# jkulhanek/viewformer

Hardware: AMD Instinct MI355X
Metric: novel views/sec (encode->AR transformer->decode), 128px 6-ctx (higher is better)
Workload: dtype bf16

## Files before the change

### viewformer_amd/csrc/epilogue.h

```cpp
#pragma once
#include "vf_common.h"

template <int EPI, bool HAS_RES, typename OffOut, typename OffRes>
__device__ __forceinline__ void vf_store_tile(const f32x16& acc, float bias, float* __restrict__ out,
                                              const float* __restrict__ res, OffOut off_out, OffRes off_res) {
    float v[16];
    if (HAS_RES) {
        float rr[16];
#pragma unroll
        for (int r = 0; r < 16; ++r) rr[r] = res[off_res(r)];
#pragma unroll
        for (int r = 0; r < 16; ++r) {
            float t = acc[r] + bias;
            if (EPI == 1) t = vf_gelu_erf(t);
            if (EPI == 2) t = vf_gelu_erf_fast(t);
            v[r] = t + rr[r];
        }
    } else {
#pragma unroll
        for (int r = 0; r < 16; ++r) {
            float t = acc[r] + bias;
            if (EPI == 1) t = vf_gelu_erf(t);
            if (EPI == 2) t = vf_gelu_erf_fast(t);
            v[r] = t;
        }
    }
#pragma unroll
    for (int r = 0; r < 16; ++r) out[off_out(r)] = v[r];
}

template <int EPI, bool HAS_RES>
__device__ __forceinline__ void vf_store_tile_ragged(const f32x16& acc, float bias, float* __restrict__ out,
                                                     const float* __restrict__ res, long long ldc, long long ldr,
                                                     int rows_left ) {
    if (rows_left <= 0) return;
    float v[16];
#pragma unroll
    for (int r = 0; r < 16; ++r) {
        const int row = (r & 3) + 8 * (r >> 2);
        float t = acc[r] + bias;
        if (EPI == 1) t = vf_gelu_erf(t);
        if (EPI == 2) t = vf_gelu_erf_fast(t);
        if (HAS_RES) t += res[(long long)(row < rows_left ? row : 0) * ldr];
        v[r] = t;
    }
#pragma unroll
    for (int r = 0; r < 16; ++r) {
        const int row = (r & 3) + 8 * (r >> 2);
        if (row < rows_left) out[(long long)row * ldc] = v[r];
    }
}

template <bool HAS_RES, typename OffOut, typename OffRes, typename Sel, typename S>
__device__ __forceinline__ void vf_store_tile_stats(const f32x16& acc, float bias, float* __restrict__ out,
                                                    const float* __restrict__ res, OffOut off_out, OffRes off_res, Sel sel,
                                                    S (&s)[2], S (&q)[2]) {
    float v[16];
    if (HAS_RES) {
        float rr[16];
#pragma unroll
        for (int r = 0; r < 16; ++r) rr[r] = res[off_res(r)];
#pragma unroll
        for (int r = 0; r < 16; ++r) v[r] = acc[r] + bias + rr[r];
    } else {
#pragma unroll
        for (int r = 0; r < 16; ++r) v[r] = acc[r] + bias;
    }
#pragma unroll
    for (int r = 0; r < 16; ++r) {
        const int k = sel(r);
        s[k] += (S)v[r];
        q[k] += (S)v[r] * (S)v[r];
    }
#pragma unroll
    for (int r = 0; r < 16; ++r) out[off_out(r)] = v[r];
}

template <typename OffOut>
__device__ __forceinline__ void vf_store_tile_pre(const f32x16& acc, float bias, float* __restrict__ out, const float (&rr)[16], OffOut off_out) {
    float v[16];
#pragma unroll
    for (int r = 0; r < 16; ++r) v[r] = acc[r] + bias + rr[r];
#pragma unroll
    for (int r = 0; r < 16; ++r) out[off_out(r)] = v[r];
}
template <typename OffOut, typename Sel, typename S>
__device__ __forceinline__ void vf_store_tile_stats_pre(const f32x16& acc, float bias, float* __restrict__ out, const float (&rr)[16], OffOut off_out,
                                                        Sel sel, S (&s)[2], S (&q)[2]) {
    float v[16];
#pragma unroll
    for (int r = 0; r < 16; ++r) v[r] = acc[r] + bias + rr[r];
#pragma unroll
    for (int r = 0; r < 16; ++r) {
        const int k = sel(r);
        s[k] += (S)v[r];
        q[k] += (S)v[r] * (S)v[r];
    }
#pragma unroll
    for (int r = 0; r < 16; ++r) out[off_out(r)] = v[r];
}

template <typename S>
__device__ __forceinline__ void vf_gn_group_reduce(S& s, S& q, int cg) {
    s += __shfl_xor(s, 32, 64);
    q += __shfl_xor(q, 32, 64);
    for (int o = 1; o < cg; o <<= 1) {
        s += __shfl_xor(s, o, 64);
        q += __shfl_xor(q, o, 64);
    }
}
```

### viewformer_amd/csrc/gemm_bf16_g256.hip

```cpp
#include "vf_common.h"
#include "epilogue.h"
#include "../../include/vf_hip.h"

namespace {

typedef __bf16 bf16x8 __attribute__((ext_vector_type(8)));
typedef __bf16 bf16x2_t __attribute__((ext_vector_type(2)));

constexpr int GM = 256, GN = 256, GK = 64;
constexpr int GA_BYTES = GM * GK * 2;
constexpr int GB_BYTES = GN * GK * 2;
constexpr int GSTAGE = GA_BYTES + GB_BYTES;

__device__ __forceinline__ void bufds16(__amdgpu_buffer_rsrc_t r, void* l, unsigned voff, unsigned soff) {
    __builtin_amdgcn_raw_ptr_buffer_load_lds(r, (__attribute__((address_space(3))) void*)l, 16, voff, soff, 0, 0);
}

template <bool DROP, int IC>
__device__ __forceinline__ void g256_store_f32(const vf_igemm_args& p, const f32x16 (&acc)[IC][2], int m_tile0, int n_tile0, int wrow0,
                                               int wave_n, int half, int l31, bool full, bool gelu) {
    const long long ldc = p.ldc, ldr = p.ldr;
    const bool has_res = p.res != nullptr;
    const bool dual = p.epilogue == VF_EPI_GELU_DUAL;
    const int odd = l31 & 1;
    const uint32_t drop_thresh = vf_dropout_thresh(p.drop_rate), drop_key = vf_dropout_key(p.drop_seed, p.drop_site, 0u);
    const float drop_scale = 1.0f / (1.0f - p.drop_rate);
#pragma unroll
    for (int j = 0; j < 2; ++j) {
        const int n = n_tile0 + wave_n * 64 + j * 32 + l31;
        const float bias = p.bias ? p.bias[n] : 0.f;
#pragma unroll
        for (int i = 0; i < IC; ++i) {
            int m0 = m_tile0 + wrow0 + i * 32 + 4 * half;
            if constexpr (DROP) asm volatile("" : "+v"(m0) :: "memory");
            const int rows_left = p.M - m0;
            float* o = p.out + (size_t)(rows_left > 0 ? m0 : 0) * ldc + n;
            float v[16];
#pragma unroll
            for (int r = 0; r < 16; ++r) v[r] = acc[i][j][r] + bias;
            if (gelu) {
#pragma unroll
                for (int r = 0; r < 16; ++r) v[r] = vf_gelu_erf_fast(v[r]);
            }
            if constexpr (DROP) {
#pragma unroll
                for (int g = 0; g < 4; ++g) {
                    const uint32_t w = vf_dropout_word(drop_key, (uint32_t)(((m0 + p.drop_row0) >> 2) + 2 * g) * (uint32_t)p.Cout + (uint32_t)n);
#pragma unroll
                    for (int e = 0; e < 4; ++e) v[4 * g + e] = vf_dropout_keep(w, e, drop_thresh) ? v[4 * g + e] * drop_scale : 0.f;
                }
            }
            if (has_res) {
                const float* rs = p.res + (size_t)(rows_left > 0 ? m0 : 0) * ldr + n;
                float rr[16];
#pragma unroll
                for (int r = 0; r < 16; ++r) {
                    const int row = (r & 3) + 8 * (r >> 2);
                    rr[r] = rs[(long long)(full || row < rows_left ? row : 0) * ldr];
                }
#pragma unroll
                for (int r = 0; r < 16; ++r) v[r] += rr[r];
            }
            if (full) {
#pragma unroll
                for (int r = 0; r < 16; ++r) o[(long long)((r & 3) + 8 * (r >> 2)) * ldc] = v[r];
            } else if (rows_left > 0) {
#pragma unroll
                for (int r = 0; r < 16; ++r) {
                    const int row = (r & 3) + 8 * (r >> 2);
                    if (row < rows_left) o[(long long)row * ldc] = v[r];
                }
            }
            if (dual) {
                __builtin_amdgcn_sched_barrier(0);
                __bf16* o16 = reinterpret_cast<__bf16*>(p.out_aux) + (size_t)(rows_left > 0 ? m0 : 0) * ldc + (n - odd);
#pragma unroll
                for (int r = 0; r < 16; ++r) v[r] = vf_gelu_erf_fast(v[r]);
#pragma unroll
                for (int r = 0; r < 16; r += 2) {
                    const float give = odd ? v[r] : v[r + 1];
                    const float got = vf_lane_xor1(give);
                    const int row = ((r + odd) & 3) + 8 * ((r + odd) >> 2);
                    bf16x2_t h;
                    h[0] = (__bf16)(odd ? got : v[r]);
                    h[1] = (__bf16)(odd ? v[r + 1] : got);
                    if (full || row < rows_left) *reinterpret_cast<bf16x2_t*>(o16 + (long long)row * ldc) = h;
                }
            }
            __builtin_amdgcn_sched_barrier(0);
        }
    }
}

template <int EPI, bool FULL, int IC>
__device__ __forceinline__ void g256_store_bf16(const vf_igemm_args& p, const f32x16 (&acc)[IC][2], int m_tile0, int n_tile0, int wrow0,
                                                int wave_n, int half, int l31) {
    __bf16* __restrict__ O = reinterpret_cast<__bf16*>(p.out);
    const int odd = l31 & 1;
#pragma unroll
    for (int j = 0; j < 2; ++j) {
        const int n = n_tile0 + wave_n * 64 + j * 32 + l31;
        const float bias = p.bias ? p.bias[n] : 0.f;
#pragma unroll
        for (int i = 0; i < IC; ++i) {
            const int m0 = m_tile0 + wrow0 + i * 32 + 4 * half;
            float t[16];
            if (EPI == 2 || EPI == 4) {
                const bool u16 = p.reserved0 & 4;
                const unsigned esz = u16 ? 2u : 4u;
                const __amdgpu_buffer_rsrc_t u_rs = __builtin_amdgcn_make_buffer_rsrc(
                    const_cast<unsigned char*>(reinterpret_cast<const unsigned char*>(p.res) + (size_t)m_tile0 * p.ldr * esz), 0,
                    (int)min((long long)0x7fffffff, (long long)(p.M - m_tile0) * p.ldr * esz), 0x00020000);
                float uu[16];
                if (u16) {
                    const unsigned voff = ((unsigned)(m0 - m_tile0) * (unsigned)p.ldr + (unsigned)(n - odd)) * 2u;
                    unsigned w[8];
#pragma unroll
                    for (int r = 0; r < 16; r += 2) {
                        const int row = ((r + odd) & 3) + 8 * ((r + odd) >> 2);
                        w[r >> 1] = __builtin_amdgcn_raw_buffer_load_b32(u_rs, voff + (unsigned)row * (unsigned)p.ldr * 2u, 0, 0);
                    }
#pragma unroll
                    for (int r = 0; r < 16; r += 2) {
                        const unsigned mine = w[r >> 1];
                        const unsigned give = odd ? (mine << 16) : (mine & 0xffff0000u);
                        const unsigned got = vf_lane_xor1(give);
                        uu[r] = __builtin_bit_cast(float, odd ? got : (mine << 16));
                        uu[r + 1] = __builtin_bit_cast(float, odd ? (mine & 0xffff0000u) : got);
                    }
                } else {
                    const unsigned voff = ((unsigned)(m0 - m_tile0) * (unsigned)p.ldr + (unsigned)n) * 4u;
#pragma unroll
                    for (int r = 0; r < 16; ++r) {
                        const unsigned soff = (unsigned)((r & 3) + 8 * (r >> 2)) * (unsigned)p.ldr * 4u;
                        uu[r] = __builtin_bit_cast(float, __builtin_amdgcn_raw_buffer_load_b32(u_rs, voff, soff, 0));
                    }
                }
                __builtin_amdgcn_sched_barrier(0);
#pragma unroll
                for (int q = 0; q < 4; ++q) {
#pragma unroll
                    for (int e = 0; e < 4; ++e)
                        t[4 * q + e] = __fmul_rn(__fadd_rn(acc[i][j][4 * q + e], bias), EPI == 4 ? uu[4 * q + e] : vf_gelu_grad_fast(uu[4 * q + e]));
                    __builtin_amdgcn_sched_barrier(0);
                }
            } else {
#pragma unroll
                for (int r = 0; r < 16; ++r) {
                    t[r] = acc[i][j][r] + bias;
                    if (EPI == 1) t[r] = vf_gelu_erf_fast(t[r]);
                }
            }
            float gq[EPI == 5 ? 16 : 1];
            if (EPI == 5) {
#pragma unroll
                for (int r = 0; r < 16; ++r) { float f, g; vf_gelu_and_grad_fast(t[r], f, g); t[r] = f; gq[r] = g; }
            }
#pragma unroll
            for (int pass = 0; pass < ((EPI == 3 || EPI == 5) ? 2 : 1); ++pass) {
                __bf16* __restrict__ dst = pass == 0 ? O : reinterpret_cast<__bf16*>(p.out_aux);
                if (EPI == 3 && pass == 1) {
                    __builtin_amdgcn_sched_barrier(0);
#pragma unroll
                    for (int r = 0; r < 16; ++r) t[r] = vf_gelu_erf_fast(t[r]);
                }
#pragma unroll
                for (int r = 0; r < 16; r += 2) {
                    const float lo = (EPI == 5 && pass == 0) ? gq[r] : t[r], hi = (EPI == 5 && pass == 0) ? gq[r + 1] : t[r + 1];
                    const float give = odd ? lo : hi;
                    const float got = vf_lane_xor1(give);
                    const int m = m0 + ((r + odd) & 3) + 8 * ((r + odd) >> 2);
                    bf16x2_t v;
                    v[0] = (__bf16)(odd ? got : lo);
                    v[1] = (__bf16)(odd ? hi : got);
                    if (FULL || m < p.M) *reinterpret_cast<bf16x2_t*>(dst + (size_t)m * p.ldc + (n - odd)) = v;
                }
            }
        }
    }
}

template <bool O16, bool DROP, int IC>
__device__ __forceinline__ void g256_tile(const vf_igemm_args& p, unsigned char* smem_b, int m_tile0, int nblk, int tid) {
    constexpr int TROWS = 2 * IC * 32;
    const int lane = tid & 63;
    const int wave = __builtin_amdgcn_readfirstlane(tid >> 6);
    const int wave_m = wave >> 2, wave_n = wave & 3;
    const int half = lane >> 5, l31 = lane & 31;
    const int wrow0 = wave_m * (IC * 32);
    const int n_tile0 = nblk * GN;
    const int nstages = p.Cin / GK;

    const bool a_mover = wave * 32 < TROWS;
    const __amdgpu_buffer_rsrc_t a_rsrc = __builtin_amdgcn_make_buffer_rsrc(const_cast<float*>(p.x), 0, 0x7fffffff, 0x00020000);
    const __amdgpu_buffer_rsrc_t w_rsrc = __builtin_amdgcn_make_buffer_rsrc(const_cast<float*>(p.w_packed), 0, 0x7fffffff, 0x00020000);
    unsigned avoff[4];
#pragma unroll
    for (int q = 0; q < 4; ++q) {
        const int r = wave * 32 + q * 8 + (lane >> 3);
        const int c = (lane & 7) ^ ((r >> 1) & 7);
        int m = m_tile0 + r;
        m = m < p.M ? m : p.M - 1;
        avoff[q] = (unsigned)(((size_t)m * p.lda) * 2 + c * 16);
    }
    const unsigned wvoff = (unsigned)((size_t)nblk * GB_BYTES + wave * 4096 + lane * 16);
    const size_t w_stage_stride = (size_t)(p.Cout / 128) * (GK * 128 * 2);
    auto issue = [&](int s) {
        unsigned char* dst = smem_b + (s & 1) * GSTAGE;
        if (IC == 4 || a_mover) {
#pragma unroll
            for (int q = 0; q < 4; ++q) bufds16(a_rsrc, dst + (wave * 32 + q * 8) * 128, avoff[q], (unsigned)(s * (GK * 2)));
        }
#pragma unroll
        for (int q = 0; q < 4; ++q) bufds16(w_rsrc, dst + GA_BYTES + wave * 4096 + q * 1024, wvoff + q * 1024, (unsigned)((size_t)s * w_stage_stride));
    };

    const unsigned a_row_off = (unsigned)((wrow0 + l31) * 128);
    const unsigned a_swz = (unsigned)((l31 >> 1) & 7);
    unsigned a_off[4];
#pragma unroll
    for (int ks = 0; ks < 4; ++ks) a_off[ks] = a_row_off + ((((unsigned)(ks * 2 + half)) ^ a_swz) << 4);
    const unsigned b_off = (unsigned)(GA_BYTES + (wave_n >> 1) * (GK * 128 * 2) + ((half * 128) + (wave_n & 1) * 64 + l31) * 16);

    f32x16 acc[IC][2];
#pragma unroll
    for (int i = 0; i < IC; ++i)
#pragma unroll
        for (int j = 0; j < 2; ++j)
#pragma unroll
            for (int r = 0; r < 16; ++r) acc[i][j][r] = 0.f;

    issue(0);
    for (int s = 0; s < nstages; ++s) {
        asm volatile("s_waitcnt vmcnt(0) lgkmcnt(0)" ::: "memory");
        __builtin_amdgcn_s_barrier();
        if (s + 1 < nstages) issue(s + 1);
        const unsigned char* buf = smem_b + (s & 1) * GSTAGE;
        bf16x8 a[2][IC], b[2][2];
        auto frags = [&](int ks, bf16x8 (&af)[IC], bf16x8 (&bf)[2]) {
#pragma unroll
            for (int j = 0; j < 2; ++j) bf[j] = *reinterpret_cast<const bf16x8*>(buf + b_off + (ks * 2 * 128 + j * 32) * 16);
#pragma unroll
            for (int i = 0; i < IC; ++i) af[i] = *reinterpret_cast<const bf16x8*>(buf + a_off[ks] + i * (32 * 128));
        };
        frags(0, a[0], b[0]);
#pragma unroll
        for (int ks = 0; ks < 4; ++ks) {
            if (ks < 3) frags(ks + 1, a[(ks + 1) & 1], b[(ks + 1) & 1]);
            __builtin_amdgcn_sched_barrier(0);
#pragma unroll
            for (int i = 0; i < IC; ++i)
#pragma unroll
                for (int j = 0; j < 2; ++j)
                    acc[i][j] = __builtin_amdgcn_mfma_f32_32x32x16_bf16(a[ks & 1][i], b[ks & 1][j], acc[i][j], 0, 0, 0);
            __builtin_amdgcn_sched_barrier(0);
        }
    }

    const bool full = m_tile0 + TROWS <= p.M;
    const bool gelu = p.epilogue == VF_EPI_GELU_ERF;
    if (O16) {
        const bool gbwd = p.epilogue == VF_EPI_GELU_BWD;
        const bool dual16 = p.epilogue == VF_EPI_GELU_DUAL;
        const bool deriv = p.reserved0 & 8;
        if (dual16 && deriv) {
            if (full) g256_store_bf16<5, true, IC>(p, acc, m_tile0, n_tile0, wrow0, wave_n, half, l31);
            else g256_store_bf16<5, false, IC>(p, acc, m_tile0, n_tile0, wrow0, wave_n, half, l31);
        } else if (gbwd && deriv) {
            if (full) g256_store_bf16<4, true, IC>(p, acc, m_tile0, n_tile0, wrow0, wave_n, half, l31);
            else g256_store_bf16<4, false, IC>(p, acc, m_tile0, n_tile0, wrow0, wave_n, half, l31);
        } else if (dual16) {
            if (full) g256_store_bf16<3, true, IC>(p, acc, m_tile0, n_tile0, wrow0, wave_n, half, l31);
            else g256_store_bf16<3, false, IC>(p, acc, m_tile0, n_tile0, wrow0, wave_n, half, l31);
        } else if (full) {
            if (gbwd) g256_store_bf16<2, true, IC>(p, acc, m_tile0, n_tile0, wrow0, wave_n, half, l31);
            else if (gelu) g256_store_bf16<1, true, IC>(p, acc, m_tile0, n_tile0, wrow0, wave_n, half, l31);
            else g256_store_bf16<0, true, IC>(p, acc, m_tile0, n_tile0, wrow0, wave_n, half, l31);
        } else {
            if (gbwd) g256_store_bf16<2, false, IC>(p, acc, m_tile0, n_tile0, wrow0, wave_n, half, l31);
            else if (gelu) g256_store_bf16<1, false, IC>(p, acc, m_tile0, n_tile0, wrow0, wave_n, half, l31);
            else g256_store_bf16<0, false, IC>(p, acc, m_tile0, n_tile0, wrow0, wave_n, half, l31);
        }
    } else {
        g256_store_f32<DROP, IC>(p, acc, m_tile0, n_tile0, wrow0, wave_n, half, l31, full, gelu);
    }
}

__device__ __forceinline__ void g256_panel_order(unsigned lbid, int mt, int nb, int& mtile, int& nblk) {
    constexpr int PANEL = 4;
    const int sn = nb <= PANEL ? nb : nb % PANEL == 0 ? PANEL : nb % 3 == 0 ? 3 : nb % 2 == 0 ? 2 : 1;
    const int per_panel = mt * sn;
    const int panel = (int)(lbid / (unsigned)per_panel);
    const int in_panel = (int)(lbid - (unsigned)panel * per_panel);
    nblk = panel * sn + in_panel % sn;
    mtile = in_panel / sn;
}

template <bool O16, bool DROP = false, bool TAIL = false>
__global__ __launch_bounds__(512, 1) void gemm_bf16_g256_kernel(vf_igemm_args p, int f_rows, int h_rows, int tail_ic) {
    extern __shared__ __attribute__((aligned(16))) unsigned char smem_b[];
    const int tid = threadIdx.x;
    const int nb = p.Cout / GN;
    int mtile, nblk;
    if constexpr (!TAIL) {
        g256_panel_order(vf_xcd_bid(), (p.M + GM - 1) / GM, nb, mtile, nblk);
        g256_tile<O16, DROP, 4>(p, smem_b, mtile * GM, nblk, tid);
    } else {
        const unsigned F = (unsigned)(f_rows * nb), tot = gridDim.x;
        const unsigned x = blockIdx.x & 7u, i = blockIdx.x >> 3;
        const unsigned nF = F / 8u + (x < (F & 7u) ? 1u : 0u);
        const unsigned baseF = x * (F / 8u) + (x < (F & 7u) ? x : (F & 7u));
        if (i < nF) {
            g256_panel_order(baseF + i, f_rows, nb, mtile, nblk);
            g256_tile<O16, DROP, 4>(p, smem_b, mtile * GM, nblk, tid);
            return;
        }
        const unsigned baseT = x * (tot / 8u) + (x < (tot & 7u) ? x : (tot & 7u));
        g256_panel_order(baseT - baseF + (i - nF), h_rows, nb, mtile, nblk);
        const int m_tile0 = f_rows * GM + mtile * (tail_ic * 64);
        if (tail_ic == 3) g256_tile<O16, DROP, 3>(p, smem_b, m_tile0, nblk, tid);
        else g256_tile<O16, DROP, 2>(p, smem_b, m_tile0, nblk, tid);
    }
}

}

struct G256Tail { int f_rows, h_rows, ic; };
static G256Tail g256_tail_policy(int M, int nb) {
    const int mt = (M + GM - 1) / GM;
    const long long ntiles = (long long)mt * nb;
    constexpr int CUS = 256;
    G256Tail none{0, 0, 0};
    if (ntiles <= CUS || !vf_selected(VF_SEL_GEMM_TAIL)) return none;
    const int last = (int)(ntiles % CUS);
    if (last == 0 || last > (CUS * 3) / 4 - 8 || last < 16) return none;
    const int f_rows = (int)((ntiles / CUS) * CUS / nb);
    if (f_rows <= 0 || f_rows >= mt) return none;
    const int rem_blocks = (M - f_rows * GM + 31) / 32;
    for (int ic = 2; ic <= 3; ++ic) {
        const int h_rows = (rem_blocks + 2 * ic - 1) / (2 * ic);
        if ((long long)h_rows * nb <= CUS) return G256Tail{f_rows, h_rows, ic};
    }
    return none;
}

int vf_gemm_bf16_g256_launch(const vf_igemm_args& a, hipStream_t stream) {
    const bool a16 = a.reserved0 & 1, o16 = a.reserved0 & 2;
    if (!a16 || a.batch > 1 || a.Cout % GN != 0 || a.Cin % GK != 0 || a.M < GM || (a.lda & 7)) return VF_ERR_UNSUPPORTED;
    if (o16 && ((a.res && a.epilogue != VF_EPI_GELU_BWD) || (a.ldc & 1))) return VF_ERR_UNSUPPORTED;
    if (a.epilogue == VF_EPI_GELU_BWD && !(o16 && a.res)) return VF_ERR_UNSUPPORTED;
    if (a.epilogue == VF_EPI_GELU_DUAL && (a.res || !a.out_aux || (a.ldc & 1))) return VF_ERR_UNSUPPORTED;
    if ((a.reserved0 & 4) && a.epilogue != VF_EPI_GELU_BWD) return VF_ERR_BAD_ARG;
    if (a.reserved0 & 8) {
        if (a.epilogue == VF_EPI_GELU_BWD ? !(a.reserved0 & 4) : !(a.epilogue == VF_EPI_GELU_DUAL && o16)) return VF_ERR_BAD_ARG;
    }
    if (a.res && a.epilogue == VF_EPI_GELU_ERF) return VF_ERR_UNSUPPORTED;
    if (a.drop_rate != 0.f && (!(a.drop_rate > 0.f && a.drop_rate < 1.f) || o16 || a.epilogue != VF_EPI_NONE || a.drop_row0 < 0 || (a.drop_row0 & 3) ||
                               (((unsigned long long)a.M + (unsigned long long)a.drop_row0 + 3) / 4) * (unsigned long long)a.Cout >= (1ull << 32)))
        return VF_ERR_UNSUPPORTED;
    if ((size_t)a.M * a.lda * 2 >= (1ull << 31) || (size_t)a.Cin * a.Cout * 2 >= (1ull << 31)) return VF_ERR_UNSUPPORTED;
    const int mt = (a.M + GM - 1) / GM, nb = a.Cout / GN;
    const G256Tail t = g256_tail_policy(a.M, nb);
    const dim3 g((unsigned)(t.f_rows ? (t.f_rows + t.h_rows) * nb : mt * nb));
    auto launch = [&](auto kernel, unsigned long long* devs) -> int {
        if (vf_attr_needed(devs)) {
            const hipError_t e = hipFuncSetAttribute(reinterpret_cast<const void*>(kernel), hipFuncAttributeMaxDynamicSharedMemorySize, 2 * GSTAGE);
            if (e != hipSuccess) return (int)e;
            vf_attr_done(devs);
        }
        hipLaunchKernelGGL(kernel, g, dim3(512), (size_t)2 * GSTAGE, stream, a, t.f_rows, t.h_rows, t.ic);
        return vf_last_status();
    };
    static unsigned long long d0 = 0, d1 = 0, d2 = 0, d3 = 0, d4 = 0, d5 = 0;
    const bool drop = a.drop_rate > 0.f;
    if (t.f_rows) {
        if (o16) return launch(gemm_bf16_g256_kernel<true, false, true>, &d3);
        return drop ? launch(gemm_bf16_g256_kernel<false, true, true>, &d5) : launch(gemm_bf16_g256_kernel<false, false, true>, &d4);
    }
    if (o16) return launch(gemm_bf16_g256_kernel<true, false, false>, &d0);
    return drop ? launch(gemm_bf16_g256_kernel<false, true, false>, &d2) : launch(gemm_bf16_g256_kernel<false, false, false>, &d1);
}
```

Before: 1165.

## Stage bf16 GEMM epilogue through LDS for coalesced 16-byte stores

Adds an epilogue path for the 256x256 bf16-output GEMM that first writes bias/GELU results into shared memory, then rereads whole rows and writes them to global memory as 16-byte vector stores. It replaces scattered 4-byte bf16x2 global stores with coalesced wide stores, and applies GELU on packed float2 vectors. The cost is extra LDS traffic and a __syncthreads per row chunk, and the path is taken only when the output is 16-byte aligned and ldc is a multiple of 8.

After: 1175, median of 6. Within noise of the previous version (+0.9%).

```diff
diff --git a/viewformer_amd/csrc/epilogue.h b/viewformer_amd/csrc/epilogue.h
--- a/viewformer_amd/csrc/epilogue.h
+++ b/viewformer_amd/csrc/epilogue.h
@@ -1,5 +1,28 @@
 #pragma once
 #include "vf_common.h"
+
+typedef float vf_f32x2 __attribute__((ext_vector_type(2)));
+__device__ __forceinline__ vf_f32x2 vf_gelu_erf_fast_pk(vf_f32x2 v) {
+    const vf_f32x2 one = 1.0f;
+    const vf_f32x2 z = __builtin_elementwise_abs(v) * 0.70710678118654752440f;
+    const vf_f32x2 d = __builtin_elementwise_fma((vf_f32x2)0.3275911f, z, one);
+    vf_f32x2 t;
+    t.x = __builtin_amdgcn_rcpf(d.x);
+    t.y = __builtin_amdgcn_rcpf(d.y);
+    vf_f32x2 p = __builtin_elementwise_fma((vf_f32x2)1.061405429f, t, (vf_f32x2)-1.453152027f);
+    p = __builtin_elementwise_fma(p, t, (vf_f32x2)1.421413741f);
+    p = __builtin_elementwise_fma(p, t, (vf_f32x2)-0.284496736f);
+    p = __builtin_elementwise_fma(p, t, (vf_f32x2)0.254829592f);
+    const vf_f32x2 a = -1.4426950408889634f * z * z;
+    vf_f32x2 e;
+    e.x = __builtin_amdgcn_exp2f(a.x);
+    e.y = __builtin_amdgcn_exp2f(a.y);
+    const vf_f32x2 erf_abs = __builtin_elementwise_fma(-p * t, e, one);
+    vf_f32x2 s;
+    s.x = copysignf(erf_abs.x, v.x);
+    s.y = copysignf(erf_abs.y, v.y);
+    return 0.5f * v * (one + s);
+}
 
 template <int EPI, bool HAS_RES, typename OffOut, typename OffRes>
 __device__ __forceinline__ void vf_store_tile(const f32x16& acc, float bias, float* __restrict__ out,
diff --git a/viewformer_amd/csrc/gemm_bf16_g256.hip b/viewformer_amd/csrc/gemm_bf16_g256.hip
--- a/viewformer_amd/csrc/gemm_bf16_g256.hip
+++ b/viewformer_amd/csrc/gemm_bf16_g256.hip
@@ -177,6 +177,60 @@
                 }
             }
         }
+    }
+}
+
+typedef unsigned u32x4 __attribute__((ext_vector_type(4)));
+template <bool GELU, int IC>
+__device__ __forceinline__ void g256_store_bf16_lds(const vf_igemm_args& p, const f32x16 (&acc)[IC][2], unsigned char* img, int m_tile0, int n_tile0,
+                                                    int wave_m, int wave_n, int half, int l31) {
+    const int odd = l31 & 1;
+    const int wrow0 = wave_m * (IC * 32);
+    float bias[2];
+#pragma unroll
+    for (int j = 0; j < 2; ++j) bias[j] = p.bias ? p.bias[n_tile0 + wave_n * 64 + j * 32 + l31] : 0.f;
+    unsigned char* const wr = img + (wrow0 + 4 * half + odd) * (GN * 2) + (wave_n * 32 + (l31 >> 1)) * 4;
+    const int frow0 = wrow0 + wave_n * 2 + half;
+    const unsigned char* const rd = img + frow0 * (GN * 2) + ((l31 ^ (half << 2)) << 4);
+    __bf16* const dst = reinterpret_cast<__bf16*>(p.out) + (size_t)(m_tile0 + frow0) * p.ldc + (n_tile0 + l31 * 8);
+    const int rows_left = p.M - (m_tile0 + frow0);
+    __syncthreads();
+#pragma unroll
+    for (int i = 0; i < IC; ++i) {
+#pragma unroll
+        for (int j = 0; j < 2; ++j) {
+            float t[16];
+            if (GELU) {
+#pragma unroll
+                for (int r = 0; r < 16; r += 2) {
+                    vf_f32x2 u;
+                    u.x = acc[i][j][r];
+                    u.y = acc[i][j][r + 1];
+                    u = vf_gelu_erf_fast_pk(u + bias[j]);
+                    t[r] = u.x;
+                    t[r + 1] = u.y;
+                }
+            } else {
+#pragma unroll
+                for (int r = 0; r < 16; ++r) t[r] = acc[i][j][r] + bias[j];
+            }
+#pragma unroll
+            for (int r = 0; r < 16; r += 2) {
+                const float give = odd ? t[r] : t[r + 1];
+                const float got = vf_lane_xor1(give);
+                bf16x2_t v;
+                v[0] = (__bf16)(odd ? got : t[r]);
+                v[1] = (__bf16)(odd ? t[r + 1] : got);
+                *reinterpret_cast<bf16x2_t*>(wr + ((j ^ odd) << 6) + (i * 32 + (r & 3) + 8 * (r >> 2)) * (GN * 2)) = v;
+            }
+        }
+        __syncthreads();
+        u32x4 q[4];
+#pragma unroll
+        for (int t = 0; t < 4; ++t) q[t] = *reinterpret_cast<const u32x4*>(rd + (i * 32 + t * 8) * (GN * 2));
+#pragma unroll
+        for (int t = 0; t < 4; ++t)
+            if (i * 32 + t * 8 < rows_left) *reinterpret_cast<u32x4*>(dst + (size_t)(i * 32 + t * 8) * p.ldc) = q[t];
     }
 }
 
@@ -272,6 +326,9 @@
         } else if (dual16) {
             if (full) g256_store_bf16<3, true, IC>(p, acc, m_tile0, n_tile0, wrow0, wave_n, half, l31);
             else g256_store_bf16<3, false, IC>(p, acc, m_tile0, n_tile0, wrow0, wave_n, half, l31);
+        } else if (!gbwd && ((p.ldc & 7) | (int)(reinterpret_cast<uintptr_t>(p.out) & 15)) == 0) {
+            if (gelu) g256_store_bf16_lds<true, IC>(p, acc, smem_b, m_tile0, n_tile0, wave_m, wave_n, half, l31);
+            else g256_store_bf16_lds<false, IC>(p, acc, smem_b, m_tile0, n_tile0, wave_m, wave_n, half, l31);
         } else if (full) {
             if (gbwd) g256_store_bf16<2, true, IC>(p, acc, m_tile0, n_tile0, wrow0, wave_n, half, l31);
             else if (gelu) g256_store_bf16<1, true, IC>(p, acc, m_tile0, n_tile0, wrow0, wave_n, half, l31);
```
